# xuxiyang1993/gym-guidance-collision-avoidance-single

Measured on NVIDIA B200. Metric: env_steps_per_sec, higher is better.
Workload: dtype f32+f64

## Files before the change

gym-guidance-collision-avoidance-single_b200/csrc/gca_abi.cu:

```cuda
#include <algorithm>
#include <climits>
#include <cmath>
#include <cstdlib>
#include <limits>
#include <map>
#include <mutex>
#include <cstring>
#include <new>
#include <string>
#include <vector>

#include "gca.h"
#include "gca_launch.h"

using namespace gca;

namespace {
thread_local std::string g_err;

int fail(int code, const std::string& msg) {
  g_err = msg;
  return code;
}

// ... 185 lines not shown
  if (!cfg) return fail(GCA_ERR_INVALID, "config is NULL");
  switch (cfg->obs_kind) {
    case GCA_OBS_VECTOR:
    case GCA_OBS_RAW: return 4 * n + 8;
    case GCA_OBS_HER:
    case GCA_OBS_DHER: return 4 * n + 6;
    case GCA_OBS_NEAREST: return 4 + 5 * cfg->nearest_n;
    case GCA_OBS_RAW6: return 6 * n + 8;
    default: return 0;
  }
}

int gca_create(const gca_config* cfg, int n_envs, int n_intruders, int mode, int draws, int device, uint64_t seed,
               uint32_t env_id0, gca_env** out) {
  if (!out) return fail(GCA_ERR_INVALID, "out is NULL");
  *out = nullptr;
  if (int rc = check_config(cfg)) return rc;
  if (n_envs <= 0 || n_intruders < 0 || n_intruders > 4096) return fail(GCA_ERR_INVALID, "n_envs must be > 0 and 0 <= n_intruders <= 4096");
  if (cfg->obs_kind == GCA_OBS_NEAREST && n_intruders <= cfg->nearest_n)
    return fail(GCA_ERR_INVALID, "GCA_OBS_NEAREST needs more intruders than nearest_n");
  if (mode != GCA_MODE_FAITHFUL && mode != GCA_MODE_FAST) return fail(GCA_ERR_INVALID, "bad mode");
  if (draws != GCA_DRAWS_TAPE && draws != GCA_DRAWS_PHILOX) return fail(GCA_ERR_INVALID, "bad draws");
  int count = 0;
  cudaError_t ce = cudaGetDeviceCount(&count);
  if (ce != cudaSuccess || count <= 0)
    return fail(GCA_ERR_CUDA, std::string("no usable CUDA device (libgca has no CPU path): ") +
                                  (ce != cudaSuccess ? cudaGetErrorString(ce) : "device count is 0"));
  if (device < 0 || device >= count) return fail(GCA_ERR_INVALID, "device index out of range");
  GCA_CUDA(cudaSetDevice(device));
  gca_env* e = new (std::nothrow) gca_env();
  if (!e) return fail(GCA_ERR_ALLOC, "out of host memory");
  e->device = device; e->mode = mode; e->draws = draws; e->cfg = *cfg; e->k = derive(*cfg); e->seed = seed; e->env_id0 = env_id0;
  e->D = gca_obs_dim(cfg, n_intruders);
  DevState& s = e->s;
  s.B = n_envs; s.N = n_intruders;
  plane_layout(s, mode == GCA_MODE_FAITHFUL);
  const size_t B = (size_t)n_envs;
  int rc = GCA_OK;
  if (!rc) rc = dev_alloc(e, &s.own_pos, B);
  if (!rc) rc = dev_alloc(e, &s.own_hs, B);
  if (!rc) rc = dev_alloc(e, &s.own_vel, B);
  if (!rc) rc = dev_alloc(e, &s.own_vel_f32, B);
  if (!rc) rc = dev_alloc(e, &s.goal, B);
  if (!rc) rc = dev_alloc(e, &s.counters, B);
  if (!rc) rc = dev_alloc(e, &s.ipos, 2 * s.pos_plane);
  if (!rc) rc = dev_alloc(e, &s.own_b, (size_t)s.T * 32);
  if (!rc) rc = dev_alloc(e, &s.ev_conf, flag_plane_words(s));
  if (!rc) rc = dev_alloc(e, &s.ev_gone, flag_plane_words(s));
  if (!rc) rc = dev_alloc(e, &s.ev_nmac, (size_t)s.T * 32);
  if (!rc) rc = dev_alloc(e, &s.ev_near, (size_t)s.T * 32);
  if (!rc) rc = dev_alloc(e, &s.pre, (size_t)s.T * 32);
  if (!rc) rc = dev_alloc(e, &s.step_seq, 1);
  if (!rc) rc = dev_alloc(e, &s.error_flag, 1);
  if (!rc) rc = dev_alloc(e, &s.ivel, vel_plane_bytes(s));
  if (!rc) rc = dev_alloc(e, &s.cflag, flag_plane_words(s));
  if (!rc) rc = dev_alloc(e, &s.dflag, mode == GCA_MODE_FAITHFUL ? flag_plane_words(s) : 1);
  if (!rc && keeps_ihs(*cfg) && n_intruders > 0) rc = dev_alloc(e, &s.ihs, (size_t)s.T * (size_t)s.N * 32);
  if (!rc) {
    std::vector<int> none((size_t)s.T * 32, INT_MAX);
    std::vector<uint32_t> inf((size_t)s.T * 32, 0x7f800000u);
    if (cudaMemcpy(s.ev_nmac, none.data(), none.size() * sizeof(int), cudaMemcpyHostToDevice) != cudaSuccess ||
        cudaMemcpy(s.ev_near, inf.data(), inf.size() * sizeof(uint32_t), cudaMemcpyHostToDevice) != cudaSuccess)
      rc = fail(GCA_ERR_CUDA, "initialising the event words failed");
  }
  if (rc) {
    gca_destroy(e);
    return rc;
  }
  *out = e;
  return GCA_OK;
}

int gca_destroy(gca_env* e) {
  if (!e) return GCA_OK;
  cudaSetDevice(e->device);
  for (void* p : e->allocs) cudaFree(p);
  for (cudaEvent_t ev : e->prof_events) cudaEventDestroy(ev);
  for (cudaEvent_t ev : e->prof_pool) cudaEventDestroy(ev);
  if (e->stream) cudaStreamDestroy(e->stream);
  if (e->copy_stream) cudaStreamDestroy(e->copy_stream);
  for (int i = 0; i < 2; ++i) {
    if (e->ev_step[i]) cudaEventDestroy(e->ev_step[i]);
    if (e->ev_copy[i]) cudaEventDestroy(e->ev_copy[i]);
  }
  delete e;
  return GCA_OK;
}

int gca_set_seed(gca_env* e, uint64_t seed) {
  if (!e) return fail(GCA_ERR_INVALID, "env is NULL");
  e->seed = seed;
  return GCA_OK;
}

int gca_set_config(gca_env* e, const gca_config* cfg) {
  if (!e) return fail(GCA_ERR_INVALID, "env is NULL");
  if (int rc = check_config(cfg)) return rc;
  if (gca_obs_dim(cfg, e->s.N) != e->D) return fail(GCA_ERR_STATE, "obs_kind change would alter the observation size");
  if (keeps_ihs(*cfg) && !e->s.ihs && e->s.N > 0)
    return fail(GCA_ERR_STATE, "the handle was created without per-intruder (heading, speed) state");
  e->cfg = *cfg;
  e->k = derive(*cfg);
  return GCA_OK;
}

int gca_reset(gca_env* e, const uint8_t* mask, const gca_tape* tape, const gca_out* out, void* stream) {
  if (!e) return fail(GCA_ERR_INVALID, "env is NULL");
  if (int rc = check_out(e, out, false)) return rc;
  if (int rc = check_tape(e, tape)) return rc;
  GCA_CUDA(cudaSetDevice(e->device));
  StepArgs a = make_args(e, nullptr, tape, out, 0);
  a.mask = mask;
  GCA_CUDA(launch_reset(e->mode == GCA_MODE_FAITHFUL, e->draws == GCA_DRAWS_TAPE, a, (cudaStream_t)stream));
  return GCA_OK;
}

int gca_step(gca_env* e, const void* actions, const gca_tape* tape, int auto_reset, const gca_out* out, void* stream) {
  if (!e) return fail(GCA_ERR_INVALID, "env is NULL");
  if (!actions) return fail(GCA_ERR_INVALID, "actions is NULL");
  if (int rc = check_out(e, out, true)) return rc;
  if (int rc = check_tape(e, tape)) return rc;
  GCA_CUDA(cudaSetDevice(e->device));
  const StepArgs a = make_args(e, actions, tape, out, auto_reset);
  cudaEvent_t* ev = nullptr;
  cudaEvent_t evs[5];
  if (e->profiling) {
    for (int i = 0; i < 5; ++i) {
      if (!e->prof_pool.empty()) {
        evs[i] = e->prof_pool.back();
        e->prof_pool.pop_back();
      } else {
        GCA_CUDA(cudaEventCreate(&evs[i]));
      }
      e->prof_events.push_back(evs[i]);
    }
    ev = evs;
  }
  GCA_CUDA(launch_step(e->mode == GCA_MODE_FAITHFUL, e->draws == GCA_DRAWS_TAPE, a, (cudaStream_t)stream, ev));
  return GCA_OK;
}

int gca_step_launches(gca_env* e) {
  if (!e) return fail(GCA_ERR_INVALID, "env is NULL");
  return step_launch_count(e->draws == GCA_DRAWS_TAPE, e->s.N, e->cfg.obs_kind, e->cfg.intruder_turns && e->s.ihs);
}

int gca_check(gca_env* e) {
  if (!e) return fail(GCA_ERR_INVALID, "env is NULL");
  GCA_CUDA(cudaSetDevice(e->device));
  GCA_CUDA(cudaDeviceSynchronize());
  int flag = 0;
  GCA_CUDA(cudaMemcpy(&flag, e->s.error_flag, sizeof(int), cudaMemcpyDeviceToHost));
  if (flag & 1) return fail(GCA_ERR_STATE, "a streaming lane timed out waiting for its ownship record (step_intruders_kernel)");
  return GCA_OK;
}

int gca_profile_enable(gca_env* e, int on) {
  if (!e) return fail(GCA_ERR_INVALID, "env is NULL");
  e->profiling = on != 0;
  return GCA_OK;
}

int gca_profile_read(gca_env* e, gca_step_profile* out) {
  if (!e || !out) return fail(GCA_ERR_INVALID, "env/out is NULL");
  GCA_CUDA(cudaSetDevice(e->device));
  GCA_CUDA(cudaDeviceSynchronize());
  gca_step_profile p = {};
  for (size_t i = 0; i + 4 < e->prof_events.size(); i += 5) {
    float ms[4];
    for (int j = 0; j < 4; ++j) GCA_CUDA(cudaEventElapsedTime(&ms[j], e->prof_events[i + j], e->prof_events[i + j + 1]));
    p.steps += 1;
    p.own_ms += ms[0]; p.intruders_ms += ms[1]; p.finish_ms += ms[2]; p.spawn_ms += ms[3];
  }
  e->prof_pool.insert(e->prof_pool.end(), e->prof_events.begin(), e->prof_events.end());
  e->prof_events.clear();
  *out = p;
  return GCA_OK;
}

int gca_observe(gca_env* e, const gca_out* out, void* stream) {
  if (!e) return fail(GCA_ERR_INVALID, "env is NULL");
  if (int rc = check_out(e, out, false)) return rc;
  GCA_CUDA(cudaSetDevice(e->device));
  const StepArgs a = make_args(e, nullptr, nullptr, out, 0);
  GCA_CUDA(launch_observe(e->mode == GCA_MODE_FAITHFUL, a, (cudaStream_t)stream));
  return GCA_OK;
}

int gca_read_counters(gca_env* e, int32_t* counters, void* stream) {
  if (!e || !counters) return fail(GCA_ERR_INVALID, "env/counters is NULL");
  GCA_CUDA(cudaSetDevice(e->device));
  GCA_CUDA(cudaMemcpyAsync(counters, e->s.counters, (size_t)e->s.B * sizeof(int4), cudaMemcpyDeviceToDevice,
                           (cudaStream_t)stream));
  return GCA_OK;
}

static void release_host_path(gca_env* e) {
  if (e->stream) cudaStreamDestroy(e->stream);
  if (e->copy_stream) cudaStreamDestroy(e->copy_stream);
  e->stream = e->copy_stream = nullptr;
  for (int i = 0; i < 2; ++i) {
    if (e->ev_step[i]) cudaEventDestroy(e->ev_step[i]);
    if (e->ev_copy[i]) cudaEventDestroy(e->ev_copy[i]);
    e->ev_step[i] = e->ev_copy[i] = nullptr;
  }
}
// ... 330 lines not shown
```

gym-guidance-collision-avoidance-single_b200/csrc/gca_device.cuh:

```cuda
#pragma once
#include <math_constants.h>

#include <cuda_runtime.h>
#include <stdint.h>

#include "gca.h"
#include "gca_math.h"

namespace gca {

struct DevState {
  float2* own_pos;
  double2* own_hs;
  double2* own_vel;
  uint8_t* own_vel_f32;
  double2* goal;
  int4* counters;
  uint8_t* ipos;
  uint8_t* ivel;
  uint32_t* cflag;
  uint32_t* dflag;
  double2* ihs;
  float4* own_b;
  uint32_t* ev_conf;
  uint32_t* ev_gone;
  int* ev_nmac;
  uint32_t* ev_near;
  uint64_t align_pad;
  double2* pre;
  uint32_t* step_seq;
  int* error_flag;
  size_t pos_plane;
  int B, N, T, U, W, Wd;
};

template <bool FAITH>
struct pos2 { using type = float2; };
template <>
struct pos2<true> { using type = double2; };

__host__ __device__ inline void plane_layout(DevState& s, bool faithful) {
  s.T = (s.B + 31) / 32;
  s.U = (s.N + 1) / 2;
  s.W = (s.N + 31) / 32;
  s.Wd = s.W > 0 ? s.W : 1;
  s.pos_plane = (size_t)s.T * (size_t)(s.U > 0 ? s.U : 1) * 512u * (faithful ? 2u : 1u);
}
__host__ __device__ inline size_t vel_plane_bytes(const DevState& s) { return (size_t)s.T * (size_t)(s.U > 0 ? s.U : 1) * 512u; }
__host__ __device__ inline size_t flag_plane_words(const DevState& s) { return (size_t)s.T * (size_t)s.Wd * 32u; }

__host__ __device__ inline size_t ipos_offset(const DevState& s, bool faithful, size_t env, int i) {
  const size_t t = env >> 5, e = env & 31;
  if (faithful) return ((t * (size_t)(2 * s.U) + (size_t)i) * 32 + e) * 16;
  return ((t * (size_t)s.U + (size_t)(i >> 1)) * 32 + e) * 16 + (size_t)(i & 1) * 8;
}
__host__ __device__ inline size_t ivel_offset(const DevState& s, size_t env, int i) {
  const size_t t = env >> 5, e = env & 31;
  return ((t * (size_t)s.U + (size_t)(i >> 1)) * 32 + e) * 16 + (size_t)(i & 1) * 8;
}
__host__ __device__ inline size_t ihs_index(const DevState& s, size_t env, int i) {
  const size_t t = env >> 5, e = env & 31;
  return (t * (size_t)s.N + (size_t)i) * 32 + e;
}
__host__ __device__ inline size_t flag_index(const DevState& s, size_t env, int w) {
  const size_t t = env >> 5, e = env & 31;
  return (t * (size_t)s.Wd + (size_t)w) * 32 + e;
}

struct Derived {
  float sep2_f, nmac2_f, init2_f;
  double sep2_d, nmac2_d, init2_d;
  double goal2_d;
  float win_w, win_h;
  float ob_w, ob_h, inv_ob_w, inv_ob_h;
  float ms, den, inv_den;
  int div1_ok;
  double dv_w, dv_h, dv_speed, dv_2pi, dv_vel, dv_shape;
  double rc_w, rc_h, rc_speed, rc_2pi, rc_vel, rc_shape;
  int ddiv_ok;
  float drift_f;
  int has_drift;
  unsigned long long turn_thresh;
};

// ... 557 lines not shown
```

gym-guidance-collision-avoidance-single_b200/csrc/gca_step.cu:

```cuda
#include <climits>
#include <cstdio>
#include <cstdlib>
#include <type_traits>
#include <utility>

#include "gca_device.cuh"
#include "gca_launch.h"
#include "gca_step_common.cuh"

namespace gca {

#ifdef GCA_PHASE_TIMING
__device__ unsigned long long g_kstamp[8];
__device__ __forceinline__ unsigned long long gtime() {
  unsigned long long t;
  asm volatile("mov.u64 %0, %%globaltimer;" : "=l"(t));
  return t;
}
__device__ unsigned long long g_cta[8192 * 2];
extern "C" int gca_debug_cta(unsigned long long* host) { return (int)cudaMemcpyFromSymbol(host, g_cta, sizeof(g_cta)); }
__device__ unsigned long long g_fin[2048 * 8];
extern "C" int gca_debug_fin(unsigned long long* host) { return (int)cudaMemcpyFromSymbol(host, g_fin, sizeof(g_fin)); }
__device__ unsigned int g_lat[8 * 64];
extern "C" int gca_debug_lat(unsigned int* host, int clear) {
  int rc = (int)cudaMemcpyFromSymbol(host, g_lat, sizeof(g_lat));
  if (clear) { static unsigned int zero[8 * 64]; rc |= (int)cudaMemcpyToSymbol(g_lat, zero, sizeof(zero)); }
  return rc;
}
#define GCA_KSTAMP_IN(kid) do { if (threadIdx.x == 0) atomicMin(&g_kstamp[2 * (kid)], gtime()); } while (0)
#define GCA_KSTAMP_OUT(kid) do { if (threadIdx.x == 0) atomicMax(&g_kstamp[2 * (kid) + 1], gtime()); } while (0)
extern "C" int gca_debug_kstamps(unsigned long long* host, int reset) {
  int rc = (int)cudaMemcpyFromSymbol(host, g_kstamp, sizeof(g_kstamp));
  if (reset) {
    unsigned long long init[8] = {~0ull, 0, ~0ull, 0, ~0ull, 0, ~0ull, ~0ull};
    rc |= (int)cudaMemcpyToSymbol(g_kstamp, init, sizeof(init));
  }
  return rc;
}
#else
#define GCA_KSTAMP_IN(kid) do { } while (0)
#define GCA_KSTAMP_OUT(kid) do { } while (0)
#endif

constexpr int kChunkUnits = 4;
constexpr int kChunkIntr = 2 * kChunkUnits;
constexpr int kTileRespawnCap = 128;
constexpr int kWarpsB = 4;
constexpr int kFaithMinBlocks = 1;
constexpr uint32_t kObsRow = 16u * kChunkIntr + 16u;
constexpr uint32_t kObsRow64 = 32u * kChunkIntr + 16u;
static_assert(32 % kChunkIntr == 0, "the event bits of a work item must not straddle a word, and the FAST write-out "
                                    "stores 32 / kChunkIntr whole env rows per instruction");
static_assert(32 * kChunkIntr == 16 * 16, "the FAITHFUL write-out stores one env's work item with 16 lanes x 16 bytes");
static_assert(kWarpsB * 32 * kObsRow64 <= 0xc000, "the FAITHFUL staging buffer must fit in static shared memory");

template <bool FAITH, bool TAPE>
__device__ __forceinline__ bool spawn_store(const StepArgs& a, Draws<TAPE>& d, uint32_t slot, size_t env, int i, int plane,
                                            float ox, float oy, real_t<FAITH>* obase) {
  const DevState& s = a.s;
  Intr<FAITH> it;
  spawn<FAITH, TAPE>(d, a.cfg, a.k, slot, ox, oy, it, ihs_slot(s, env, i));
  store_ipos<FAITH>(s, plane, env, i, it);
  store_ivel(s, env, i, it.vx, it.vy);
  write_obs_intruder<FAITH>(a, obase, i, it);
  return it.is64;
}

template <bool FAITH>
__device__ __forceinline__ void spawn_reset_word(const StepArgs& a, Draws<false>& d, size_t env, int r, int lane, int plane,
                                                 const float2& own) {
  const DevState& s = a.s;
  const int i = r * 32 + lane;
  bool wide = false;
  if (i < s.N)
// ... 426 lines not shown
        const double p = d.next();
        if (!(p < c.turn_prob)) continue;
        const double raw = d.next();
        double2 ih = s.ihs[ihs_index(s, me, i)];
        double sn, cs;
        ih.x = __dadd_rn(ih.x, __dmul_rn(raw, 3.141592653589793 / 180.0));
        gca_sincos(ih.x, &sn, &cs);
        s.ihs[ihs_index(s, me, i)] = ih;
        store_ivel(s, me, i, (float)__dmul_rn(ih.y, cs), (float)__dmul_rn(ih.y, sn));
      }
    }
  }
#ifdef GCA_PHASE_TIMING
  fin_t3 = gtime();
#endif
  const bool resets = a.auto_reset && has_env && done;
  int reset_slot = -1;
  if constexpr (TAPE) {
    reset_envs_warp<FAITH, TAPE>(a, env0, lane, resets, nxt, d, pos, hs, vel, goal);
  } else {
    const uint32_t rmask = __ballot_sync(FULL, resets);
    if (rmask) {
      int base = 0;
      if (lane == 0) base = atomicAdd(&bs->count, __popc(rmask));
      base = __shfl_sync(FULL, base, 0);
      if (resets) {
        reset_slot = base + __popc(rmask & ((1u << lane) - 1u));
        bs->env[reset_slot] = (int)me;
        draw_goal(d, c, goal.x, goal.y);
      }
#ifdef GCA_PHASE_TIMING
      fin_resets += __popc(rmask);
#endif
    }
  }
  if (resets) {
    if constexpr (!TAPE) {
      reset_ownship<TAPE>(c, d, pos, hs, vel);
      if (reset_slot >= 0) {
        bs->pos[reset_slot] = pos;
        bs->tick[reset_slot] = cnt.z;
      }
    }
    cnt.w += 1;
    store_own_reset<FAITH>(a, me, pos, hs, vel, goal, cnt);
  }
  if (has_env) {
    cnt.z += 1;
    s.counters[me] = cnt;
    if constexpr (TAPE) a.cursor[me] = d.cur;
  }
#ifdef GCA_PHASE_TIMING
  if (lane == 0 && tile < 2048) {
    g_fin[tile * 8 + 0] = fin_t0; g_fin[tile * 8 + 1] = gtime(); g_fin[tile * 8 + 3] = fin_resets;
    g_fin[tile * 8 + 4] = fin_t1; g_fin[tile * 8 + 5] = fin_t2; g_fin[tile * 8 + 6] = fin_t3;
  }
#endif
}

template <bool FAITH>
__device__ __forceinline__ void spawn_phase(const StepArgs& a, const int tile, const int wib, const int lane,
                                            WarpScratch* ws, BlockScratch* bs) {
  const DevState& s = a.s;
  Draws<false> d;
  d.k0 = a.key0; d.k1 = a.key1;
  if (tile < s.T) {
    __syncwarp();
    const int n_resp = ws->n_jobs;
    for (int at = lane; at < n_resp; at += 32) {
      const uint32_t rec = ws->list[at];
      const int e = (int)(rec >> 8), i = (int)(rec & 0xffu);
      const int tick = ws->tick[e];
      if (tick < 0) continue;
      const size_t env = (size_t)tile * 32 + e;
      const float2 own = ws->pos[e];
      d.env = a.env_id0 + (uint32_t)env;
      d.tick = (uint32_t)tick;
      const bool is64 = spawn_store<FAITH, false>(a, d, (uint32_t)i, env, i, (tick & 1) ^ 1, own.x, own.y,
                                                  obs_intruder_base<FAITH>(a, env));
      if constexpr (FAITH) {
        if (is64) atomicOr(&s.dflag[flag_index(s, env, i >> 5)], 1u << (i & 31));
      }
    }
  }
#ifdef GCA_PHASE_TIMING
  if (lane == 0 && tile < 2048 && tile < s.T) {
    g_fin[tile * 8 + 2] = ws->n_jobs;
    g_fin[tile * 8 + 7] = gtime();
  }
#endif
  __syncthreads();
  const int rounds = s.W, total = bs->count * rounds;
  for (int job = wib; job < total; job += 4) {
    const size_t env = (size_t)bs->env[job / rounds];
    const int r = job % rounds;
    const int tick = bs->tick[job / rounds];
    d.env = a.env_id0 + (uint32_t)env;
    d.tick = (uint32_t)tick;
    spawn_reset_word<FAITH>(a, d, env, r, lane, (tick & 1) ^ 1, bs->pos[job / rounds]);
  }
}

template <bool FAITH, bool TAPE>
__global__ void __launch_bounds__(128) step_finish_kernel(const __grid_constant__ StepArgs a) {
  __shared__ WarpScratch ws[TAPE ? 1 : 4];
  __shared__ BlockScratch bs;
  if (!TAPE && threadIdx.x == 0) bs.count = 0;
  pdl_wait();
  GCA_KSTAMP_IN(2);
  const int wib = threadIdx.x >> 5, lane = threadIdx.x & 31;
  const long long tile = (long long)blockIdx.x * 4 + wib;
  if constexpr (TAPE) {
    if (tile < a.s.T) finish_tile<FAITH, TAPE>(a, (int)tile, lane, nullptr, nullptr);
  } else {
    __syncthreads();
    if (tile < a.s.T) finish_tile<FAITH, TAPE>(a, (int)tile, lane, &ws[wib], &bs);
    if (a.s.N > 0) spawn_phase<FAITH>(a, (int)(tile < a.s.T ? tile : a.s.T), wib, lane, &ws[wib], &bs);
    if (blockIdx.x == 0 && threadIdx.x == 0) *a.s.step_seq += 1u;
  }
  GCA_KSTAMP_OUT(2);
}

template <bool FAITH, int MINB>
__global__ void __launch_bounds__(128, MINB) step_n0_kernel(const __grid_constant__ StepArgs a) {
  __shared__ WarpScratch ws[4];
  __shared__ BlockScratch bs;
  if (threadIdx.x == 0) bs.count = 0;
  pdl_wait();
  __syncthreads();
  const int wib = threadIdx.x >> 5, lane = threadIdx.x & 31;
  const long long tile = (long long)blockIdx.x * 4 + wib;
  const size_t me = (size_t)tile * 32 + lane;
  if (me < (size_t)a.s.B) own_update<FAITH, false>(a, me, 0u, false);
  if (tile < a.s.T) finish_tile<FAITH, false>(a, (int)tile, lane, &ws[wib], &bs);
}

template <bool FAITH, int OM, bool DRIFT = false>
__global__ void __launch_bounds__(kWarpsB * 32, FAITH ? kFaithMinBlocks : 1) step_intruders_kernel(const __grid_constant__ StepArgs a) {
  static_assert(!(DRIFT && OM), "a handle with a position drift takes the generic observation path");
  pdl_wait();
  GCA_KSTAMP_IN(1);
#ifdef GCA_PHASE_TIMING
  if (threadIdx.x == 0 && blockIdx.x < 8192) g_cta[2 * blockIdx.x] = gtime();
#endif
  using R = real_t<FAITH>;
  static_assert(!(FAITH && OM), "the specialised observation path is FAST only");
  constexpr uint32_t kWarpSmem = OM ? 32 * kObsRow : (FAITH ? 32 * kObsRow64 : 16);
  constexpr uint32_t kStageBytes = kWarpsB * kWarpSmem;
  __shared__ __align__(16) uint8_t stage_smem[kStageBytes];
  const DevState& s = a.s;
  const Derived& k = a.k;
  uint32_t stamp = 0u;
  if (a.own_blocks > 0) {
    stamp = *s.step_seq + 1u;
    if (blockIdx.x < (unsigned)a.own_blocks) {
      GCA_KSTAMP_IN(0);
      const size_t env = (size_t)((stamp & 1u) ? (unsigned)a.own_blocks - 1u - blockIdx.x : blockIdx.x) * (kWarpsB * 32) + threadIdx.x;
      if (env < (size_t)s.B) {
        own_update<FAITH, false>(a, env, stamp, true);
      } else if (env < (size_t)s.T * 32) {
        st_release_quad(reinterpret_cast<float*>(&s.own_b[env]), 0.f, 0.f, 0.f, __uint_as_float(stamp));
      }
      GCA_KSTAMP_OUT(0);
      return;
    }
  }
  const int lane = threadIdx.x & 31, wib = threadIdx.x >> 5;
  const int n_chunks = (s.U + kChunkUnits - 1) / kChunkUnits;
  const long long work = (long long)(blockIdx.x - (unsigned)a.own_blocks) * kWarpsB + wib;
  do {
  if (work >= (long long)s.T * n_chunks) break;
  const int tile_fwd = (int)(work / n_chunks), ch = (int)(work - (long long)tile_fwd * n_chunks);
  const int tile = (a.own_blocks > 0 && (stamp & 1u)) ? s.T - 1 - tile_fwd : tile_fwd;
  const size_t me = (size_t)tile * 32 + lane;
  const bool has_env = me < (size_t)s.B;
  const int u0 = ch * kChunkUnits, i0 = 2 * u0;
  const int n_here = min(kChunkIntr, s.N - i0);
  constexpr size_t kPosUnits = FAITH ? 2 : 1;
  const size_t unit0 = (size_t)tile * s.U + u0;
  const uint8_t* vsrc = s.ivel + (unit0 * 32 + lane) * 16;
  const uint64_t pol = l2_evict_first_policy();
  float4 vv[kChunkUnits];
  const bool full = !FAITH && n_here == kChunkIntr;
  if (full) {
#pragma unroll
    for (int g = 0; g < kChunkUnits; ++g) vv[g] = ldg_stream(vsrc + g * 512, pol);
  }
  float4 ob;
  GCA_KSTAMP_IN(3);
  if (a.own_blocks > 0) {
    int spins = 0;
    for (;;) {
      ob = ld_volatile_f4(&s.own_b[me]);
      if (__all_sync(FULL, __float_as_uint(ob.w) == stamp)) break;
      if (++spins > (1 << 22)) {
        if (lane == 0) atomicExch(s.error_flag, 1);
        break;
      }
      __nanosleep(32);
    }
  } else {
    ob = s.own_b[me];
  }
#ifdef GCA_PHASE_TIMING
  if (threadIdx.x == 0) { atomicMin(&g_kstamp[7], gtime()); }
#endif
  const uint32_t bits = __float_as_uint(ob.z);
  const bool runs = (bits & kOwnRuns) != 0;
  const int par = (bits & kOwnPlane) ? 1 : 0;
  const float ox = ob.x, oy = ob.y;
  const size_t pos_off = (unit0 * kPosUnits * 32 + lane) * 16;
  const uint8_t* psrc = s.ipos + (size_t)par * s.pos_plane + pos_off;
  uint8_t* pdst = s.ipos + (size_t)(par ^ 1) * s.pos_plane + pos_off;
  R* obase = obs_intruder_base<FAITH>(a, me);
  uint32_t gone = 0, conf = 0, nmac = 0;
  float near2 = __uint_as_float(0x7f800000u);

  bool fast_done = false;
  if constexpr (!FAITH) {
    if (full) {
      fast_done = true;
      float4 p[kChunkUnits], np[kChunkUnits];
#ifdef GCA_PHASE_TIMING
      const long long lat_t0 = clock64();
#endif
#pragma unroll
      for (int g = 0; g < kChunkUnits; ++g) p[g] = ldg_stream(psrc + g * 512, pol);
#ifdef GCA_PHASE_TIMING
      {
        float sink = 0.f;
        for (int g = 0; g < kChunkUnits; ++g) sink += p[g].x + p[g].w;
        if (__any_sync(FULL, sink == 1.2345e38f)) atomicAdd(&g_lat[0], 1u);
        const long long dt = clock64() - lat_t0;
        if (lane == 0) atomicAdd(&g_lat[min(7, tile_fwd * 8 / s.T) * 64 + (int)min(63ll, dt >> 6)], 1u);
      }
#endif
      const uint32_t wbits = __float_as_uint(k.win_w), hbits = __float_as_uint(k.win_h);
#pragma unroll
      for (int g = 0; g < kChunkUnits; ++g) {
        float4 dv = vv[g];
        if constexpr (DRIFT)
          dv = make_float4(__fadd_rn(dv.x, k.drift_f), __fadd_rn(dv.y, k.drift_f), __fadd_rn(dv.z, k.drift_f),
                           __fadd_rn(dv.w, k.drift_f));
        np[g] = make_float4(__fadd_rn(p[g].x, dv.x), __fadd_rn(p[g].y, dv.y),
                            __fadd_rn(p[g].z, dv.z), __fadd_rn(p[g].w, dv.w));
        const bool oob0 = (__float_as_uint(np[g].x) > wbits) | (__float_as_uint(np[g].y) > hbits);
        const bool oob1 = (__float_as_uint(np[g].z) > wbits) | (__float_as_uint(np[g].w) > hbits);
        gone |= ((oob0 ? 1u : 0u) | (oob1 ? 2u : 0u)) << (2 * g);
        const float d0 = dist2_f32(ox, oy, np[g].x, np[g].y), d1 = dist2_f32(ox, oy, np[g].z, np[g].w);
// ... 106 lines not shown
        const size_t row_off = (own_first(a.cfg) ? 6 : 0) + 4 * (size_t)i0;
#pragma unroll 4
        for (int it2 = 0; it2 < 16; ++it2) {
          const int e = sub + 2 * it2;
          const size_t env_e = (size_t)tile * 32 + e;
          if (env_e < (size_t)s.B) {
            const double2 val = *reinterpret_cast<const double2*>(stg + e * kObsRow64 + piece * 16);
            double* dst = reinterpret_cast<double*>(a.obs) + env_e * (size_t)a.D + row_off + 2 * (size_t)piece;
            *reinterpret_cast<double2*>(dst) = val;
          }
        }
      }
    }
  }
  if (!fast_done && has_env) {
    uint32_t dw = 0;
    if constexpr (FAITH) dw = s.dflag[flag_index(s, me, i0 >> 5)] >> (i0 & 31);
    for (int j = 0; j < n_here; ++j) {
      const int i = i0 + j;
      Intr<FAITH> it;
      const float2 v = *reinterpret_cast<const float2*>(vsrc + (j >> 1) * 512 + (j & 1) * 8);
      it.vx = v.x; it.vy = v.y;
      if constexpr (FAITH) {
        const double2 q = *reinterpret_cast<const double2*>(psrc + j * 512);
        it.px = q.x; it.py = q.y;
        it.is64 = (dw >> j) & 1u;
      } else {
        const float2 q = *reinterpret_cast<const float2*>(psrc + (j >> 1) * 512 + (j & 1) * 8);
        it.px = q.x; it.py = q.y;
      }
      if (runs) {
        const bool oob = advance<FAITH, DRIFT>(k, it);
        bool lt_sep, lt_nmac, lt_init;
        separation<FAITH>(k, ox, oy, it, lt_sep, lt_nmac, lt_init);
        gone |= (oob ? 1u : 0u) << j;
        conf |= (lt_sep ? 1u : 0u) << j;
        nmac |= (lt_nmac ? 1u : 0u) << j;
        if constexpr (!FAITH) near2 = fminf(near2, dist2_f32(ox, oy, it.px, it.py));
      }
      if constexpr (FAITH) *reinterpret_cast<double2*>(pdst + j * 512) = make_double2(it.px, it.py);
      else *reinterpret_cast<float2*>(pdst + (j >> 1) * 512 + (j & 1) * 8) = make_float2(it.px, it.py);
      write_obs_intruder<FAITH>(a, obase, i, it);
    }
  }
  if (has_env) {
    const size_t fi = flag_index(s, me, i0 >> 5);
    if (gone) atomicOr(&s.ev_gone[fi], gone << (i0 & 31));
    if (conf) atomicOr(&s.ev_conf[fi], conf << (i0 & 31));
    nmac &= conf;
    if (nmac) atomicMin(&s.ev_nmac[me], i0 + __ffs(nmac) - 1);
    if constexpr (!FAITH) {
      if (a.cfg.shaped_nearest && runs) atomicMin(&s.ev_near[me], __float_as_uint(near2));
    }
  }
  } while (0);
#ifdef GCA_PHASE_TIMING
  __syncthreads();
  if (threadIdx.x == 0 && blockIdx.x < 8192) g_cta[2 * blockIdx.x + 1] = gtime();
#endif
  GCA_KSTAMP_OUT(1);
}

template <bool FAITH, bool TAPE>
__global__ void __launch_bounds__(128) reset_kernel(const StepArgs a) {
  const DevState& s = a.s;
  const int lane = threadIdx.x & 31;
  const long long tile = (long long)blockIdx.x * 4 + (threadIdx.x >> 5);
  if (tile >= s.T) return;
  const size_t env0 = (size_t)tile * 32;
  const bool has_env = env0 + lane < (size_t)s.B;
  const size_t me = has_env ? env0 + lane : env0;
  const bool selected = has_env && (a.mask == nullptr || a.mask[me] != 0);
  int4 cnt = make_int4(0, 0, 0, 0);
  if (has_env) cnt = s.counters[me];
  Draws<TAPE> d = make_draws<TAPE>(a, me, (uint32_t)cnt.z);
  const int nxt = (cnt.z & 1) ^ 1;
  float2 pos = make_float2(0.f, 0.f);
  double2 hs = make_double2(0., 0.), vel = make_double2(0., 0.), goal = make_double2(0., 0.);
  reset_envs_warp<FAITH, TAPE>(a, env0, lane, selected, nxt, d, pos, hs, vel, goal);
  if (selected) {
    store_own_reset<FAITH>(a, me, pos, hs, vel, goal, cnt);
    cnt.z += 1;
    s.counters[me] = cnt;
    if constexpr (TAPE) a.cursor[me] = d.cur;
    if (a.done) a.done[me] = 0;
    if (a.info) a.info[me] = 0;
  }
}

template <bool FAITH>
__global__ void __launch_bounds__(128) observe_kernel(const StepArgs a) {
  const DevState& s = a.s;
  const size_t me = (size_t)blockIdx.x * 128 + threadIdx.x;
  if (me >= (size_t)s.B) return;
  const int plane = s.counters[me].z & 1;
  real_t<FAITH>* obase = obs_intruder_base<FAITH>(a, me);
  for (int i = 0; i < s.N; ++i) {
    Intr<FAITH> it;
    load_intruder<FAITH>(s, plane, me, i, it);
    write_obs_intruder<FAITH>(a, obase, i, it);
  }
  const float2 pos = s.own_pos[me];
  const double2 hs = s.own_hs[me], vel = s.own_vel[me], goal = s.goal[me];
  write_obs_own<FAITH>(a, me, pos.x, pos.y, vel.x, vel.y, s.own_vel_f32[me] != 0, hs.x, hs.y, goal.x, goal.y);
}

// ... 63 lines not shown
        const double2 ih = s.ihs ? s.ihs[ihs_index(s, me, i)] : make_double2(0.0, 0.0);
        V2* o = stage + lane * kRowStride + 3 * (i - i0);
        o[0] = V2{(R)px[h], (R)py[h]};
        o[1] = V2{(R)vx[h], (R)vy[h]};
        o[2] = V2{(R)ih.y, (R)ih.x};
      }
    }
  }
  if (!TURN && !obs) return;
  __syncthreads();
  if constexpr (TURN) {
    for (int k = threadIdx.x; k < turn_count; k += 128) {
      const int e = turn_list[k] >> 3, i = i0 + (turn_list[k] & 7);
      const size_t env = (size_t)tile * 32 + e;
      Draws<false> d;
      d.k0 = a.key0; d.k1 = a.key1;
      d.env = a.env_id0 + (uint32_t)env;
      d.tick = (uint32_t)s.counters[env].z - 1u;
      double uu, unused, sn, cs;
      d.uniform2(GCA_SLOT_TURN | (uint32_t)i, 1u, uu, unused);
      const double raw = __dadd_rn(-c.turn_max_deg, __dmul_rn(__dadd_rn(c.turn_max_deg, c.turn_max_deg), uu));
      double2 ih = s.ihs[ihs_index(s, env, i)];
      ih.x = __dadd_rn(ih.x, __dmul_rn(raw, 3.141592653589793 / 180.0));
      gca_sincos(ih.x, &sn, &cs);
      const float nvx = (float)__dmul_rn(ih.y, cs), nvy = (float)__dmul_rn(ih.y, sn);
      s.ihs[ihs_index(s, env, i)] = ih;
      store_ivel(s, env, i, nvx, nvy);
      if (obs) {
        V2* o = stage + e * kRowStride + 3 * (i - i0);
        o[1] = V2{(R)nvx, (R)nvy};
        o[2] = V2{(R)ih.y, (R)ih.x};
      }
    }
    if (!obs) return;
    __syncthreads();
  }
  const int n_here = min(kTurnIntr, s.N - i0);
  const int row_v2 = 3 * n_here;
  for (int idx = threadIdx.x; idx < 32 * kRowV2; idx += 128) {
    const int e = idx / kRowV2, j = idx - e * kRowV2;
    const size_t env = (size_t)tile * 32 + e;
    if (j < row_v2 && env < (size_t)s.B) {
      R* dst = reinterpret_cast<R*>(a.obs) + env * (size_t)a.D + 6 * (size_t)i0;
      reinterpret_cast<V2*>(dst)[j] = stage[e * kRowStride + j];
    }
  }
}

static bool has_turn_pass(const StepArgs& a) {
  return a.s.N > 0 && (a.cfg.obs_kind == GCA_OBS_RAW6 || (a.cfg.intruder_turns && a.s.ihs));
}
static unsigned turn_blocks(const DevState& s) { return (unsigned)((size_t)s.T * (size_t)((s.N + kTurnIntr - 1) / kTurnIntr)); }

template <bool FAITH, bool TAPE>
static cudaError_t launch_step_t(const StepArgs& a0, cudaStream_t st, cudaEvent_t* ev) {
  StepArgs a = a0;
  const DevState& s = a.s;
  const unsigned env_blocks = (unsigned)(((size_t)s.T * 32 + 127) / 128);
  cudaStreamCaptureStatus cap = cudaStreamCaptureStatusNone;
  if (ev) cudaStreamIsCapturing(st, &cap);
  auto mark = [&](int i) {
    if (!ev) return;
    if (cap == cudaStreamCaptureStatusActive) cudaEventRecordWithFlags(ev[i], st, cudaEventRecordExternal);
    else cudaEventRecord(ev[i], st);
  };
  mark(0);
  a.own_blocks = 0;
  if constexpr (TAPE) launch_pdl(step_own_kernel<FAITH, TAPE>, env_blocks, 128, st, a);
  mark(1);
  if (!TAPE && s.N == 0) {
    if constexpr (!TAPE) {
      if (s.B > (1 << 18)) launch_pdl(step_n0_kernel<FAITH, 8>, env_blocks, 128, st, a);
      else launch_pdl(step_n0_kernel<FAITH, 1>, env_blocks, 128, st, a);
    }
    mark(2);
    mark(3);
    mark(4);
    return cudaGetLastError();
  }
  if (s.N > 0) {
    const int n_chunks = (s.U + kChunkUnits - 1) / kChunkUnits;
    a.own_blocks = TAPE ? 0 : (int)(((size_t)s.T * 32 + kWarpsB * 32 - 1) / (kWarpsB * 32));
    const unsigned blocks = (unsigned)(((long long)s.T * n_chunks + kWarpsB - 1) / kWarpsB) + (unsigned)a.own_blocks;
    if constexpr (FAITH) {
      if (a.k.has_drift) launch_pdl(step_intruders_kernel<true, 0, true>, blocks, kWarpsB * 32, st, a);
      else launch_pdl(step_intruders_kernel<true, 0>, blocks, kWarpsB * 32, st, a);
    } else {
      const bool own_first = a.cfg.obs_kind == GCA_OBS_HER || a.cfg.obs_kind == GCA_OBS_DHER;
      const bool special = a.k.div1_ok && !a.k.has_drift;
      if (special && a.cfg.obs_kind == GCA_OBS_VECTOR) launch_pdl(step_intruders_kernel<false, 1>, blocks, kWarpsB * 32, st, a);
      else if (special && own_first) launch_pdl(step_intruders_kernel<false, 2>, blocks, kWarpsB * 32, st, a);
      else if (a.k.has_drift) launch_pdl(step_intruders_kernel<false, 0, true>, blocks, kWarpsB * 32, st, a);
      else launch_pdl(step_intruders_kernel<false, 0>, blocks, kWarpsB * 32, st, a);
    }
  }
  mark(2);
  launch_pdl(step_finish_kernel<FAITH, TAPE>, (unsigned)((s.T + 3) / 4), 128, st, a);
  mark(3);
  if (a.cfg.obs_kind == GCA_OBS_NEAREST)
    launch_pdl(nearest_obs_kernel<FAITH>, (unsigned)(((size_t)s.B + 31) / 32), 128, st, a);
  if (has_turn_pass(a)) launch_pdl(turn_obs_kernel<FAITH, !TAPE>, turn_blocks(s), 128, st, a);
  mark(4);
  return cudaGetLastError();
}

cudaError_t launch_step(bool faith, bool tape, const StepArgs& a, cudaStream_t st, cudaEvent_t* ev) {
  if (faith) return tape ? launch_step_t<true, true>(a, st, ev) : launch_step_t<true, false>(a, st, ev);
  return tape ? launch_step_t<false, true>(a, st, ev) : launch_step_t<false, false>(a, st, ev);
}

int step_launch_count(bool tape, int n_intruders, int obs_kind, bool turns) {
  if (!tape && n_intruders == 0) return 1 + (obs_kind == GCA_OBS_NEAREST ? 1 : 0);
  return (tape ? 2 : 1) + (n_intruders > 0 ? 1 : 0) + (obs_kind == GCA_OBS_NEAREST ? 1 : 0) +
         (n_intruders > 0 && (obs_kind == GCA_OBS_RAW6 || turns) ? 1 : 0);
}

cudaError_t launch_reset(bool faith, bool tape, const StepArgs& a, cudaStream_t st) {
  const unsigned blocks = (unsigned)((a.s.T + 3) / 4);
  if (faith) {
    if (tape) reset_kernel<true, true><<<blocks, 128, 0, st>>>(a);
    else reset_kernel<true, false><<<blocks, 128, 0, st>>>(a);
  } else {
    if (tape) reset_kernel<false, true><<<blocks, 128, 0, st>>>(a);
    else reset_kernel<false, false><<<blocks, 128, 0, st>>>(a);
  }
  if (a.cfg.obs_kind == GCA_OBS_NEAREST) return launch_observe(faith, a, st);
  if (a.cfg.obs_kind == GCA_OBS_RAW6 && a.s.N > 0) {
    if (faith) turn_obs_kernel<true, false><<<turn_blocks(a.s), 128, 0, st>>>(a);
    else turn_obs_kernel<false, false><<<turn_blocks(a.s), 128, 0, st>>>(a);
  }
  return cudaGetLastError();
}

cudaError_t launch_observe(bool faith, const StepArgs& a, cudaStream_t st) {
  const unsigned blocks = (unsigned)(((size_t)a.s.B + 127) / 128);
  if (a.cfg.obs_kind == GCA_OBS_NEAREST) {
    const unsigned nb = (unsigned)(((size_t)a.s.B + 31) / 32);
    if (faith) nearest_obs_kernel<true><<<nb, 128, 0, st>>>(a);
    else nearest_obs_kernel<false><<<nb, 128, 0, st>>>(a);
  } else if (faith) observe_kernel<true><<<blocks, 128, 0, st>>>(a);
  else observe_kernel<false><<<blocks, 128, 0, st>>>(a);
  if (a.cfg.obs_kind == GCA_OBS_RAW6 && a.s.N > 0) {
    if (faith) turn_obs_kernel<true, false><<<turn_blocks(a.s), 128, 0, st>>>(a);
    else turn_obs_kernel<false, false><<<turn_blocks(a.s), 128, 0, st>>>(a);
  }
  return cudaGetLastError();
}
// ... 3 lines not shown
```

gym-guidance-collision-avoidance-single_b200/csrc/gca_step_common.cuh:

```cuda
#pragma once
#include <utility>

#include "gca_device.cuh"

namespace gca {

constexpr uint32_t kOwnRuns = 1u;
constexpr uint32_t kOwnPlane = 2u;

__device__ __forceinline__ void pdl_wait() { asm volatile("griddepcontrol.wait;" ::: "memory"); }

template <bool TAPE>
__device__ __forceinline__ void reset_ownship(const gca_config& c, Draws<TAPE>& d, float2& pos, double2& hs, double2& vel) {
  double sn, cs;
  if (c.random_start) {
    double x, y, speed, heading;
    draw_pos(d, c, GCA_SLOT_OWN_RESET, GCA_BLOCK_POS, x, y);
    draw_speed_heading(d, c, GCA_SLOT_OWN_RESET, speed, heading);
    pos = make_float2((float)x, (float)y);
    hs = make_double2(heading, speed);
  } else {
    pos = make_float2(50.0f, 50.0f);
    hs = make_double2(3.141592653589793 / 4, c.min_speed);
  }
  gca_sincos(hs.x, &sn, &cs);
  vel = make_double2((double)(float)__dmul_rn(hs.y, cs), (double)(float)__dmul_rn(hs.y, sn));
}

template <bool TAPE>
__device__ __forceinline__ Draws<TAPE> make_draws(const StepArgs& a, size_t me, uint32_t tick) {
  Draws<TAPE> d;
  if constexpr (TAPE) {
    d.tape = a.tape + me * (size_t)a.tape_stride;
    d.cur = a.cursor[me];
  } else {
    d.k0 = a.key0; d.k1 = a.key1;
    d.env = a.env_id0 + (uint32_t)me;
    d.tick = tick;
  }
  return d;
}

struct Settled {
  double reward;
  int info;
  int done;
};
__device__ __forceinline__ Settled settle_own(const gca_config& c, const Derived& k, bool maxstep_hit, float2 pos, double2 goal) {
  double reward;
  int info, done = 0;
  if (maxstep_hit) {
    reward = 0.0; done = 1; info = GCA_INFO_MAXSTEPS;
  } else if (c.wall_kind != GCA_WALL_NONE && !in_map_f32(k, pos.x, pos.y)) {
    reward = c.r_wall; done = c.wall_kind == GCA_WALL_TERMINAL; info = GCA_INFO_WALL;
  } else {
    const double dg = dist_f64((double)pos.x, (double)pos.y, goal.x, goal.y);
    if (dg < c.goal_radius) {
      reward = c.r_goal; done = 1; info = GCA_INFO_GOAL;
    } else {
      reward = c.shaped_default ? ddiv_prepared(k, -dg, k.dv_shape, k.rc_shape) : c.r_default;
      info = GCA_INFO_NONE;
    }
  }
// ... 29 lines not shown
```

Baseline: 1.560 billion.

## Overlap finish kernel with intruder streaming via per-tile readiness counters

```diff
diff --git a/gym-guidance-collision-avoidance-single_b200/csrc/gca_abi.cu b/gym-guidance-collision-avoidance-single_b200/csrc/gca_abi.cu
--- a/gym-guidance-collision-avoidance-single_b200/csrc/gca_abi.cu
+++ b/gym-guidance-collision-avoidance-single_b200/csrc/gca_abi.cu
@@ -261,6 +261,8 @@
   if (!rc) rc = dev_alloc(e, &s.pre, (size_t)s.T * 32);
   if (!rc) rc = dev_alloc(e, &s.step_seq, 1);
   if (!rc) rc = dev_alloc(e, &s.error_flag, 1);
+  if (!rc) rc = dev_alloc(e, &s.tile_ready, (size_t)s.T);
+  if (!rc) rc = dev_alloc(e, &s.finish_exits, 1);
   if (!rc) rc = dev_alloc(e, &s.ivel, vel_plane_bytes(s));
   if (!rc) rc = dev_alloc(e, &s.cflag, flag_plane_words(s));
   if (!rc) rc = dev_alloc(e, &s.dflag, mode == GCA_MODE_FAITHFUL ? flag_plane_words(s) : 1);
@@ -361,6 +363,7 @@
   int flag = 0;
   GCA_CUDA(cudaMemcpy(&flag, e->s.error_flag, sizeof(int), cudaMemcpyDeviceToHost));
   if (flag & 1) return fail(GCA_ERR_STATE, "a streaming lane timed out waiting for its ownship record (step_intruders_kernel)");
+  if (flag & 2) return fail(GCA_ERR_STATE, "a finish warp timed out waiting for its tile's work items (step_finish_kernel)");
   return GCA_OK;
 }
 
diff --git a/gym-guidance-collision-avoidance-single_b200/csrc/gca_device.cuh b/gym-guidance-collision-avoidance-single_b200/csrc/gca_device.cuh
--- a/gym-guidance-collision-avoidance-single_b200/csrc/gca_device.cuh
+++ b/gym-guidance-collision-avoidance-single_b200/csrc/gca_device.cuh
@@ -30,6 +30,8 @@
   double2* pre;
   uint32_t* step_seq;
   int* error_flag;
+  uint32_t* tile_ready;
+  uint32_t* finish_exits;
   size_t pos_plane;
   int B, N, T, U, W, Wd;
 };
diff --git a/gym-guidance-collision-avoidance-single_b200/csrc/gca_step.cu b/gym-guidance-collision-avoidance-single_b200/csrc/gca_step.cu
--- a/gym-guidance-collision-avoidance-single_b200/csrc/gca_step.cu
+++ b/gym-guidance-collision-avoidance-single_b200/csrc/gca_step.cu
@@ -19,7 +19,8 @@
 }
 __device__ unsigned long long g_cta[8192 * 2];
 extern "C" int gca_debug_cta(unsigned long long* host) { return (int)cudaMemcpyFromSymbol(host, g_cta, sizeof(g_cta)); }
-__device__ unsigned long long g_fin[2048 * 8];
+constexpr int kFinStamps = 10;
+__device__ unsigned long long g_fin[2048 * kFinStamps];
 extern "C" int gca_debug_fin(unsigned long long* host) { return (int)cudaMemcpyFromSymbol(host, g_fin, sizeof(g_fin)); }
 __device__ unsigned int g_lat[8 * 64];
 extern "C" int gca_debug_lat(unsigned int* host, int clear) {
@@ -552,8 +553,8 @@
   }
 #ifdef GCA_PHASE_TIMING
   if (lane == 0 && tile < 2048) {
-    g_fin[tile * 8 + 0] = fin_t0; g_fin[tile * 8 + 1] = gtime(); g_fin[tile * 8 + 3] = fin_resets;
-    g_fin[tile * 8 + 4] = fin_t1; g_fin[tile * 8 + 5] = fin_t2; g_fin[tile * 8 + 6] = fin_t3;
+    g_fin[tile * kFinStamps + 0] = fin_t0; g_fin[tile * kFinStamps + 1] = gtime(); g_fin[tile * kFinStamps + 3] = fin_resets;
+    g_fin[tile * kFinStamps + 4] = fin_t1; g_fin[tile * kFinStamps + 5] = fin_t2; g_fin[tile * kFinStamps + 6] = fin_t3;
   }
 #endif
 }
@@ -585,8 +586,8 @@
   }
 #ifdef GCA_PHASE_TIMING
   if (lane == 0 && tile < 2048 && tile < s.T) {
-    g_fin[tile * 8 + 2] = ws->n_jobs;
-    g_fin[tile * 8 + 7] = gtime();
+    g_fin[tile * kFinStamps + 2] = ws->n_jobs;
+    g_fin[tile * kFinStamps + 7] = gtime();
   }
 #endif
   __syncthreads();
@@ -601,22 +602,59 @@
   }
 }
 
+__device__ __forceinline__ void wait_tile(const DevState& s, int tile, int lane, uint32_t stamp, int n_chunks) {
+  if (lane == 0) {
+    const uint32_t target = stamp * (uint32_t)(n_chunks + 1);
+    int spins = 0;
+    for (;;) {
+      uint32_t v;
+      asm volatile("ld.relaxed.gpu.global.u32 %0, [%1];" : "=r"(v) : "l"(s.tile_ready + tile) : "memory");
+      if ((int32_t)(v - target) >= 0) break;
+      if (++spins > (1 << 22)) {
+        atomicOr(s.error_flag, 2);
+        break;
+      }
+      __nanosleep(32);
+    }
+    asm volatile("fence.acq_rel.gpu;" ::: "memory");
+  }
+  __syncwarp();
+}
+
 template <bool FAITH, bool TAPE>
 __global__ void __launch_bounds__(128) step_finish_kernel(const __grid_constant__ StepArgs a) {
   __shared__ WarpScratch ws[TAPE ? 1 : 4];
   __shared__ BlockScratch bs;
-  if (!TAPE && threadIdx.x == 0) bs.count = 0;
-  pdl_wait();
-  GCA_KSTAMP_IN(2);
+  __shared__ uint32_t stamp_sh;
   const int wib = threadIdx.x >> 5, lane = threadIdx.x & 31;
-  const long long tile = (long long)blockIdx.x * 4 + wib;
   if constexpr (TAPE) {
+    pdl_wait();
+    GCA_KSTAMP_IN(2);
+    const long long tile = (long long)blockIdx.x * 4 + wib;
     if (tile < a.s.T) finish_tile<FAITH, TAPE>(a, (int)tile, lane, nullptr, nullptr);
   } else {
+    if (threadIdx.x == 0) {
+      bs.count = 0;
+      stamp_sh = *a.s.step_seq + 1u;
+    }
     __syncthreads();
-    if (tile < a.s.T) finish_tile<FAITH, TAPE>(a, (int)tile, lane, &ws[wib], &bs);
+    GCA_KSTAMP_IN(2);
+    const uint32_t stamp = stamp_sh;
+    const unsigned blk = (stamp & 1u) ? gridDim.x - 1u - blockIdx.x : blockIdx.x;
+    const long long tile = (long long)blk * 4 + wib;
+    if (tile < a.s.T) {
+#ifdef GCA_PHASE_TIMING
+      if (lane == 0 && tile < 2048) g_fin[tile * kFinStamps + 9] = gtime();
+#endif
+      wait_tile(a.s, (int)tile, lane, stamp, (a.s.U + kChunkUnits - 1) / kChunkUnits);
+      finish_tile<FAITH, TAPE>(a, (int)tile, lane, &ws[wib], &bs);
+    }
     if (a.s.N > 0) spawn_phase<FAITH>(a, (int)(tile < a.s.T ? tile : a.s.T), wib, lane, &ws[wib], &bs);
-    if (blockIdx.x == 0 && threadIdx.x == 0) *a.s.step_seq += 1u;
+    pdl_wait();
+    if (threadIdx.x == 0 && atomicAdd(a.s.finish_exits, 1u) == gridDim.x - 1u) {
+      *a.s.finish_exits = 0u;
+      *a.s.step_seq = stamp;
+    }
   }
   GCA_KSTAMP_OUT(2);
 }
@@ -639,6 +677,7 @@
 __global__ void __launch_bounds__(kWarpsB * 32, FAITH ? kFaithMinBlocks : 1) step_intruders_kernel(const __grid_constant__ StepArgs a) {
   static_assert(!(DRIFT && OM), "a handle with a position drift takes the generic observation path");
   pdl_wait();
+  if (a.own_blocks > 0) pdl_trigger();
   GCA_KSTAMP_IN(1);
 #ifdef GCA_PHASE_TIMING
   if (threadIdx.x == 0 && blockIdx.x < 8192) g_cta[2 * blockIdx.x] = gtime();
@@ -661,6 +700,8 @@
       } else if (env < (size_t)s.T * 32) {
         st_release_quad(reinterpret_cast<float*>(&s.own_b[env]), 0.f, 0.f, 0.f, __uint_as_float(stamp));
       }
+      const size_t tile = env >> 5;
+      if (tile < (size_t)s.T) tile_signal(&s.tile_ready[tile], threadIdx.x & 31);
       GCA_KSTAMP_OUT(0);
       return;
     }
@@ -694,7 +735,7 @@
       ob = ld_volatile_f4(&s.own_b[me]);
       if (__all_sync(FULL, __float_as_uint(ob.w) == stamp)) break;
       if (++spins > (1 << 22)) {
-        if (lane == 0) atomicExch(s.error_flag, 1);
+        if (lane == 0) atomicOr(s.error_flag, 1);
         break;
       }
       __nanosleep(32);
@@ -907,6 +948,12 @@
     if constexpr (!FAITH) {
       if (a.cfg.shaped_nearest && runs) atomicMin(&s.ev_near[me], __float_as_uint(near2));
     }
+  }
+  if (a.own_blocks > 0) {
+    tile_signal(&s.tile_ready[me >> 5], threadIdx.x & 31);
+#ifdef GCA_PHASE_TIMING
+    if (lane == 0 && tile < 2048) atomicMax(&g_fin[tile * kFinStamps + 8], gtime());
+#endif
   }
   } while (0);
 #ifdef GCA_PHASE_TIMING
@@ -1076,6 +1123,11 @@
 }
 static unsigned turn_blocks(const DevState& s) { return (unsigned)((size_t)s.T * (size_t)((s.N + kTurnIntr - 1) / kTurnIntr)); }
 
+constexpr int kStepCarveoutPercent = 72;
+static void prefer_step_carveout(void (*kernel)(StepArgs)) {
+  cudaFuncSetAttribute(reinterpret_cast<const void*>(kernel), cudaFuncAttributePreferredSharedMemoryCarveout, kStepCarveoutPercent);
+}
+
 template <bool FAITH, bool TAPE>
 static cudaError_t launch_step_t(const StepArgs& a0, cudaStream_t st, cudaEvent_t* ev) {
   StepArgs a = a0;
@@ -1106,17 +1158,22 @@
     const int n_chunks = (s.U + kChunkUnits - 1) / kChunkUnits;
     a.own_blocks = TAPE ? 0 : (int)(((size_t)s.T * 32 + kWarpsB * 32 - 1) / (kWarpsB * 32));
     const unsigned blocks = (unsigned)(((long long)s.T * n_chunks + kWarpsB - 1) / kWarpsB) + (unsigned)a.own_blocks;
+    void (*stream_kernel)(StepArgs);
     if constexpr (FAITH) {
-      if (a.k.has_drift) launch_pdl(step_intruders_kernel<true, 0, true>, blocks, kWarpsB * 32, st, a);
-      else launch_pdl(step_intruders_kernel<true, 0>, blocks, kWarpsB * 32, st, a);
+      stream_kernel = a.k.has_drift ? step_intruders_kernel<true, 0, true> : step_intruders_kernel<true, 0>;
     } else {
       const bool own_first = a.cfg.obs_kind == GCA_OBS_HER || a.cfg.obs_kind == GCA_OBS_DHER;
       const bool special = a.k.div1_ok && !a.k.has_drift;
-      if (special && a.cfg.obs_kind == GCA_OBS_VECTOR) launch_pdl(step_intruders_kernel<false, 1>, blocks, kWarpsB * 32, st, a);
-      else if (special && own_first) launch_pdl(step_intruders_kernel<false, 2>, blocks, kWarpsB * 32, st, a);
-      else if (a.k.has_drift) launch_pdl(step_intruders_kernel<false, 0, true>, blocks, kWarpsB * 32, st, a);
-      else launch_pdl(step_intruders_kernel<false, 0>, blocks, kWarpsB * 32, st, a);
-    }
+      if (special && a.cfg.obs_kind == GCA_OBS_VECTOR) stream_kernel = step_intruders_kernel<false, 1>;
+      else if (special && own_first) stream_kernel = step_intruders_kernel<false, 2>;
+      else if (a.k.has_drift) stream_kernel = step_intruders_kernel<false, 0, true>;
+      else stream_kernel = step_intruders_kernel<false, 0>;
+    }
+    if constexpr (!TAPE) {
+      prefer_step_carveout(stream_kernel);
+      prefer_step_carveout(step_finish_kernel<FAITH, TAPE>);
+    }
+    launch_pdl(stream_kernel, blocks, kWarpsB * 32, st, a);
   }
   mark(2);
   launch_pdl(step_finish_kernel<FAITH, TAPE>, (unsigned)((s.T + 3) / 4), 128, st, a);
diff --git a/gym-guidance-collision-avoidance-single_b200/csrc/gca_step_common.cuh b/gym-guidance-collision-avoidance-single_b200/csrc/gca_step_common.cuh
--- a/gym-guidance-collision-avoidance-single_b200/csrc/gca_step_common.cuh
+++ b/gym-guidance-collision-avoidance-single_b200/csrc/gca_step_common.cuh
@@ -9,6 +9,12 @@
 constexpr uint32_t kOwnPlane = 2u;
 
 __device__ __forceinline__ void pdl_wait() { asm volatile("griddepcontrol.wait;" ::: "memory"); }
+__device__ __forceinline__ void pdl_trigger() { asm volatile("griddepcontrol.launch_dependents;" ::: "memory"); }
+
+__device__ __forceinline__ void tile_signal(uint32_t* counter, int lane) {
+  __syncwarp();
+  if (lane == 0) asm volatile("red.release.gpu.global.add.u32 [%0], 1;" ::"l"(counter) : "memory");
+}
 
 template <bool TAPE>
 __device__ __forceinline__ void reset_ownship(const gca_config& c, Draws<TAPE>& d, float2& pos, double2& hs, double2& vel) {
```

Result: slower. 1.397 billion (median of 6 runs) (-10.4%).
